# p768lwy3/torecsys

Measured on AMD Instinct MI355X. Metric: CTR samples/sec fwd+bwd (DeepFM, 39 fields x dim 64), higher is better.
Workload: dtype bf16; 1 GPU; BASELINE.json configs[1]: DeepFM 39 Criteo-shaped fields, MLP [400,400,400], 1000000 total rows, embed_dim 64, batch 65536, uniform indices, uniform field sizes; global_batch=65536, rows=1000000, parallelism=single, microbatches=1, optimizer=none, hipgraph=True, hipgraph_input_sets=1, hipgraph_steps_per_replay=4, fused_lookup_fm=True

## Files before the change

### include/trs_abi.h

```cpp
#ifndef TRS_ABI_H_
#define TRS_ABI_H_

#include <stddef.h>
#include <stdint.h>

#ifdef __cplusplus
extern "C" {
#endif

#define TRS_ABI_VERSION 3

enum { TRS_F32 = 0, TRS_BF16 = 1 };
enum { TRS_I64 = 0, TRS_I32 = 1 };
enum {
  TRS_OK = 0,
  TRS_EINVAL = -1,
  TRS_EDTYPE = -2,
  TRS_ESHAPE = -3,
  TRS_EALIGN = -4,
  TRS_ELAUNCH = -5,
  TRS_EWORKSPACE = -6
};

typedef void* trs_stream_t;
// ... 413 lines not shown
                      int64_t B, int32_t L, const void* w_qk, const void* b_qk, int32_t H, int32_t mode,
                      const void* gout, void* dx, float* dw_part, float* db_part, int32_t blocks, void* workspace,
                      size_t ws_bytes, int32_t* err_flag, trs_stream_t stream);

int trs_attn_pool_ragged_blocks(int64_t B, int32_t max_len, int32_t E, int32_t H, int32_t dtype, int32_t backward);
size_t trs_attn_pool_ragged_bwd_workspace_bytes(int32_t blocks, int32_t max_len, int32_t E, int32_t H);
int trs_attn_pool_ragged_fwd(const void* table, int64_t V, int32_t E, int32_t dtype, const void* ids, int32_t ids_dtype,
                             int64_t n, const void* offsets, int32_t off_dtype, int64_t n_off, int64_t B, int32_t max_len,
                             int64_t exclude_row, const void* w_qk, const void* b_qk, int32_t H, int32_t mode, void* out,
                             float* cnt, int32_t* err_flag, trs_stream_t stream);
int trs_attn_pool_ragged_bwd(const void* table, int64_t V, int32_t E, int32_t dtype, const void* ids, int32_t ids_dtype,
                             int64_t n, const void* offsets, int32_t off_dtype, int64_t n_off, int64_t B, int32_t max_len,
                             int64_t exclude_row, const void* w_qk, const void* b_qk, int32_t H, int32_t mode,
                             const void* gout, void* dx, float* dw_part, float* db_part, int32_t blocks, void* workspace,
                             size_t ws_bytes, int32_t* err_flag, trs_stream_t stream);

int trs_self_attn_path(int32_t L, int32_t E, int32_t H, int32_t dtype);
int trs_self_attn_blocks(int64_t B, int32_t L, int32_t E, int32_t H, int32_t dtype, int32_t backward);
size_t trs_self_attn_bwd_workspace_bytes(int32_t blocks, int32_t E);
int trs_self_attn_fwd(const void* x, int64_t B, int32_t L, int32_t E, int32_t H, int32_t dtype, const void* w_in,
                      const void* b_in, const void* w_out, const void* b_out, void* y, trs_stream_t stream);
int trs_self_attn_bwd(const void* x, int64_t B, int32_t L, int32_t E, int32_t H, int32_t dtype, const void* w_in,
                      const void* b_in, const void* w_out, const void* b_out, const void* gout, void* dx,
                      void* workspace, size_t ws_bytes, int32_t blocks, trs_stream_t stream);

int trs_dynamic_routing_path(int32_t N, int32_t R, int32_t K, int32_t dtype);
int trs_dynamic_routing_fwd(const float* priors, const void* noise, int64_t B, int32_t N, int32_t R, int32_t K,
                            int32_t num_iter, int32_t dtype, void* out, float* c_out, float* z_out, trs_stream_t stream);
int trs_dynamic_routing_bwd(const void* noise, const float* c, const float* z, const void* gout, int64_t B, int32_t N,
                            int32_t R, int32_t K, int32_t dtype, void* dpri, trs_stream_t stream);

int trs_seq_rnn_path(int32_t cell, int32_t L, int32_t E, int32_t dtype);
size_t trs_seq_rnn_workspace_bytes(int32_t cell, int32_t E);
int trs_seq_rnn_fwd(const void* table, int64_t V, int32_t E, int32_t dtype, const void* idx, int32_t idx_dtype,
                    const void* lengths, int32_t len_dtype, int64_t B, int32_t L, const void* w_ih, const void* w_hh,
                    const void* b_ih, const void* b_hh, int32_t cell, int32_t mode, int32_t average, float* scale,
                    void* out, void* h_save, float* c_save, void* workspace, size_t ws_bytes, int32_t* err_flag,
                    trs_stream_t stream);
int trs_seq_rnn_bwd(const void* table, int64_t V, int32_t E, int32_t dtype, const void* idx, int32_t idx_dtype,
                    const void* lengths, int32_t len_dtype, int64_t B, int32_t L, const void* w_ih, const void* w_hh,
                    const void* b_ih, const void* b_hh, int32_t cell, int32_t mode, const float* scale,
                    const void* h_save, const float* c_save, const void* gout, void* dgates, void* dgates_h,
                    void* workspace, size_t ws_bytes, trs_stream_t stream);

int trs_pack_columns(const void* const* srcs, const int32_t* widths, int32_t nsrc, int32_t src_dtype,
                     int64_t B, void* out, int32_t out_dtype, trs_stream_t stream);

int trs_ctr_logit_fwd(const void* fm, int32_t E, const void* feat, int32_t N, const void* const* extras,
                      const int64_t* extra_strides, int32_t n_extras, const void* bias, int64_t B, int32_t dtype,
                      void* out, trs_stream_t stream);
size_t trs_bce_logits_workspace_bytes(int64_t B);
int trs_bce_logits_fwd(const void* logits, int32_t dtype, const void* labels, int32_t label_dtype, int64_t B, float* loss,
                       void* workspace, size_t ws_bytes, trs_stream_t stream);
int trs_bce_logits_bwd(const void* logits, int32_t dtype, const void* labels, int32_t label_dtype, const float* gout,
                       int64_t B, void* glogits, trs_stream_t stream);

int trs_pair_score_path(int32_t E, int32_t dtype);
int trs_embed_pair_score_fwd(const void* a_table, int64_t Va, const void* a_idx, int64_t a_offset, const void* t_table,
                             int64_t Vt, const void* t_idx, int64_t t_offset, int32_t E, int32_t dtype, int32_t idx_dtype,
                             int64_t B, int32_t K, int32_t sim, void* scores, int32_t out_dtype, int32_t* err_flag,
                             trs_stream_t stream);
size_t trs_pair_score_bwd_workspace_bytes(int64_t B, int32_t K, int32_t E, int32_t dtype);
int trs_embed_pair_score_bwd(const void* a_table, int64_t Va, const void* a_idx, int64_t a_offset, const void* t_table,
                             int64_t Vt, const void* t_idx, int64_t t_offset, int32_t E, int32_t dtype, int32_t idx_dtype,
                             int64_t B, int32_t K, int32_t sim, const void* g_scores, int32_t g_dtype, void* g_block,
                             void* workspace, size_t ws_bytes, trs_stream_t stream);

size_t trs_rank_loss_workspace_bytes(int64_t B);
int trs_rank_loss_fwd(const void* pos, int64_t pos_stride, const void* neg, int64_t neg_stride, int32_t dtype,
                      const void* mask, int64_t B, int32_t K, int32_t kind, float margin, int32_t reduction, float* loss,
                      float* denom, void* workspace, size_t ws_bytes, trs_stream_t stream);
int trs_rank_loss_bwd(const void* pos, int64_t pos_stride, const void* neg, int64_t neg_stride, int32_t dtype,
                      const void* mask, int64_t B, int32_t K, int32_t kind, float margin, int32_t reduction,
                      const float* gout, const float* denom, void* g_pos, int64_t g_pos_stride, void* g_neg,
                      int64_t g_neg_stride, trs_stream_t stream);

#ifdef __cplusplus
}
#endif
#endif
```

### torecsys_amd/_abi.py

```python
from __future__ import annotations

import ctypes
import os
import threading
from ctypes import c_char_p, c_int32, c_int64, c_size_t, c_void_p

import torch

_HERE = os.path.dirname(os.path.abspath(__file__))
LIB_PATH = os.environ.get("TRS_LIB_PATH") or os.path.join(_HERE, "libtrs_hip.so")

TRS_F32, TRS_BF16 = 0, 1
TRS_I64, TRS_I32 = 0, 1

_P, _I32, _I64, _SZ, _F32 = c_void_p, c_int32, c_int64, c_size_t, ctypes.c_float

_OPTIMIZER_TAIL = [_I32, _F32, _P, _F32, _F32, _F32, _P, _P, _P, _SZ, _P]
_SR_TAIL = [ctypes.c_uint64, ctypes.c_uint64, _P]

SIGNATURES = {
    "trs_version": (c_int32, []),
    "trs_last_error_string": (c_char_p, []),
    "trs_rowdot_fwd": (c_int32, [_P, _P, _P, _I64, _I32, _I32, _P, _P]),
    "trs_rowdot_bwd_workspace_bytes": (_SZ, [_I64, _I32]),
# ... 123 lines not shown
    "trs_senet_scale_fwd": (c_int32, [_P, _P, _I64, _I32, _I32, _I32, _P, _P]),
    "trs_senet_scale_bwd": (c_int32, [_P, _P, _P, _P, _I64, _I32, _I32, _I32, _P, _P, _P]),
    "trs_moe_gate_vector_shape": (c_int32, [_I32, _I32]),
    "trs_moe_gate_last_path": (c_int32, []),
    "trs_moe_gate_fwd": (c_int32, [_P, _P, _P, _I64, _I32, _I32, _I32, _P, _P]),
    "trs_moe_gate_bwd": (c_int32, [_P, _P, _P, _P, _I64, _I32, _I32, _I32, _P, _P, _P]),
    "trs_dynamic_routing_path": (c_int32, [_I32, _I32, _I32, _I32]),
    "trs_dynamic_routing_fwd": (c_int32, [_P, _P, _I64, _I32, _I32, _I32, _I32, _I32, _P, _P, _P, _P]),
    "trs_dynamic_routing_bwd": (c_int32, [_P, _P, _P, _P, _I64, _I32, _I32, _I32, _I32, _P, _P]),
    "trs_seq_rnn_path": (c_int32, [_I32, _I32, _I32, _I32]),
    "trs_seq_rnn_workspace_bytes": (_SZ, [_I32, _I32]),
    "trs_seq_rnn_fwd": (c_int32, [_P, _I64, _I32, _I32, _P, _I32, _P, _I32, _I64, _I32, _P, _P, _P, _P, _I32, _I32, _I32, _P,
                                  _P, _P, _P, _P, _SZ, _P, _P]),
    "trs_seq_rnn_bwd": (c_int32, [_P, _I64, _I32, _I32, _P, _I32, _P, _I32, _I64, _I32, _P, _P, _P, _P, _I32, _I32, _P, _P,
                                  _P, _P, _P, _P, _P, _SZ, _P]),
    "trs_fm_fwd": (c_int32, [_P, _I64, _I32, _I32, _I32, _P, _P, _P]),
    "trs_fm_bwd": (c_int32, [_P, _P, _P, _I64, _I32, _I32, _I32, _P, _P]),
    "trs_pair_dot_fwd": (c_int32, [_P, _I64, _I32, _I32, _I32, _P, _P]),
    "trs_embed_pair_dot": (c_int32, [_P, _I64, _I32, _I32, _P, _I32, _P, _I64, _I32, _P, _P, _P, _P]),
    "trs_pair_dot_bwd": (c_int32, [_P, _P, _I64, _I32, _I32, _I32, _P, _P]),
    "trs_ffm_fwd": (c_int32, [_P, _I64, _I32, _I32, _I32, _P, _P]),
    "trs_ffm_bwd": (c_int32, [_P, _P, _I64, _I32, _I32, _I32, _P, _P]),
    "trs_ffm_fused_fwd": (c_int32, [_P, _I64, _I32, _I32, _P, _I32, _P, _I64, _I32, _P, _P, _P]),
    "trs_ffm_fused_bwd": (c_int32, [_P, _I64, _I32, _I32, _P, _I32, _P, _P, _P, _P, _I64, _I32, _P, _P, _P]),
    "trs_cross_workspace_bytes": (_SZ, [_I64, _I32, _I32, _I32]),
    "trs_cross_fwd": (c_int32, [_P, _P, _P, _I64, _I32, _I32, _I32, _P, _P, _SZ, _P]),
    "trs_cross_bwd": (c_int32, [_P, _P, _P, _P, _I64, _I32, _I32, _I32, _I32, _P, _P, _P, _P, _SZ, _P]),
    "trs_cin_fwd": (c_int32, [_P, _P, _P, _P, _I64, _I32, _I32, _I32, _I32, _I32, _P, _P, _P]),
    "trs_cin_bwd": (c_int32, [_P, _P, _P, _P, _I64, _I32, _I32, _I32, _I32, _I32, _P, _P, _P, _I32, _P]),
    "trs_cin_cl_workspace_bytes": (_SZ, [_I32, _I32, _I32]),
    "trs_cin_cl_fwd": (c_int32, [_P, _I32, _P, _I32, _P, _P, _I64, _I32, _I32, _I32, _I32, _I32, _I32, _P, _P, _SZ, _P]),
    "trs_cin_cl_bwd_data_workspace_bytes": (_SZ, [_I32, _I32, _I32]),
    "trs_cin_cl_bwd_data": (c_int32, [_P, _I32, _P, _I32, _P, _I32, _P, _I64, _I32, _I32, _I32, _I32, _I32, _I32, _P, _P,
                                      _I32, _P, _SZ, _P]),
    "trs_cin_dw_workspace_bytes": (_SZ, [_I64, _I32, _I32, _I32]),
    "trs_cin_dw": (c_int32, [_P, _I64, _P, _P, _I64, _I32, _I32, _I32, _I32, _I32, _I32, _P, _P, _SZ, _P]),
    "trs_relu_bwd_bias_workspace_bytes": (_SZ, [_I64, _I32]),
    "trs_relu_bwd_bias": (c_int32, [_P, _P, _I64, _I32, _I32, _P, _P, _P, _SZ, _P]),
    "trs_mlp_fused_supported": (c_int32, [_I32, _P]),
    "trs_mlp_fused_family": (c_int32, [_I32, _P, _I64, _I32]),
    "trs_mlp_fused_workspace_bytes": (_SZ, [_I32, _P]),
    "trs_mlp_fused_mask_bytes": (_SZ, [_I64]),
    "trs_mlp_fused_fwd": (c_int32, [_P, _I64, _I32, _P, _P, _P, _P, _P, _P, _P, _I32, _I32, _I32, _P, _SZ, _P]),
    "trs_mlp_fused_bwd_data": (c_int32, [_P, _I64, _I32, _P, _P, _P, _P, _P, _P, _P, _P, _I32, _I32, _P, _SZ, _P]),
    "trs_mlp_fused_bwd_wlast_part_bytes": (_SZ, [_I32, _P, _I64, _I32, _I32, _I32]),
    "trs_mlp_fused_bwd_data_wlast": (c_int32, [_P, _I32, _I64, _I32, _P, _P, _P, _P, _P, _P, _P, _P, _P, _I32, _I32, _P, _SZ, _P,
                                               _I32, _I32, _P, _SZ, _P]),
    "trs_mlp_fused_bwd_data_parts": (c_int32, [_P, _I32, _I64, _I32, _P, _P, _P, _P, _P, _P, _P, _I32, _I32, _P, _SZ, _P, _P,
                                               _P, _I32, _I32, _P, _SZ, _P]),
    "trs_colsum_parts_reduce": (c_int32, [_I32, _P, _P, _P, _I32, _P, _P]),
    "trs_ctr_logit_fwd": (c_int32, [_P, _I32, _P, _I32, _P, _P, _I32, _P, _I64, _I32, _P, _P]),
    "trs_bce_logits_workspace_bytes": (_SZ, [_I64]),
    "trs_bce_logits_fwd": (c_int32, [_P, _I32, _P, _I32, _I64, _P, _P, _SZ, _P]),
    "trs_bce_logits_bwd": (c_int32, [_P, _I32, _P, _I32, _P, _I64, _P, _P]),
    "trs_pair_score_path": (c_int32, [_I32, _I32]),
    "trs_embed_pair_score_fwd": (c_int32, [_P, _I64, _P, _I64, _P, _I64, _P, _I64, _I32, _I32, _I32, _I64, _I32, _I32, _P,
                                           _I32, _P, _P]),
    "trs_pair_score_bwd_workspace_bytes": (_SZ, [_I64, _I32, _I32, _I32]),
    "trs_embed_pair_score_bwd": (c_int32, [_P, _I64, _P, _I64, _P, _I64, _P, _I64, _I32, _I32, _I32, _I64, _I32, _I32, _P,
                                           _I32, _P, _P, _SZ, _P]),
    "trs_rank_loss_workspace_bytes": (_SZ, [_I64]),
    "trs_rank_loss_fwd": (c_int32, [_P, _I64, _P, _I64, _I32, _P, _I64, _I32, _I32, _F32, _I32, _P, _P, _P, _SZ, _P]),
    "trs_rank_loss_bwd": (c_int32, [_P, _I64, _P, _I64, _I32, _P, _I64, _I32, _I32, _F32, _I32, _P, _P, _P, _I64, _P, _I64,
                                    _P]),
    "trs_bucket_workspace_bytes": (_SZ, [_I64, _I32]),
    "trs_bucket_by_owner": (c_int32, [_P, _I32, _P, _I64, _I32, _I64, _I32, _P, _P, _P, _P, _P, _SZ, _P]),
    "trs_embed_fm_sharded": (c_int32, [_P, _I64, _P, _I64, _I64, _I32, _I32, _P, _P, _I32, _I32, _I64, _I32, _P, _P, _P, _P,
                                       _P]),
    "trs_permute_grad": (c_int32, [_P, _P, _P, _P, _P, _I64, _I32, _I32, _I32, _P, _P]),
    "trs_bag_route_count": (c_int32, [_P, _I32, _I64, _I32, _I64, _I64, _I32, _P, _P, _P]),
    "trs_bag_route_place": (c_int32, [_P, _I32, _I64, _I32, _I64, _I64, _I32, _P, _P, _I64, _P]),
    "trs_bag_pool_segments": (c_int32, [_P, _I64, _I32, _I32, _P, _I64, _P, _I64, _P, _P, _P]),
    "trs_bag_combine": (c_int32, [_P, _I32, _I64, _I32, _F32, _I32, _P, _P]),
    "trs_bag_expand_grad": (c_int32, [_P, _I32, _I32, _P, _I64, _P, _I64, _I64, _I64, _P, _P, _P]),
}

_lib = None
_lock = threading.Lock()


def load() -> ctypes.CDLL:
    global _lib
    if _lib is not None:
        return _lib
    with _lock:
        if _lib is not None:
            return _lib
        if not os.path.exists(LIB_PATH):
            raise RuntimeError(
                f"torecsys_amd: HIP library not built ({LIB_PATH} missing). Run "
                "`python -m torecsys_amd.build` (or __graft_entry__.build()). There is no CPU fallback.")
        lib = ctypes.CDLL(LIB_PATH)
        for name, (res, args) in SIGNATURES.items():
            try:
                fn = getattr(lib, name)
            except AttributeError as e:
                raise RuntimeError(f"torecsys_amd: {LIB_PATH} does not export {name}; rebuild it") from e
            fn.restype = res
            fn.argtypes = args
        _lib = lib
    return _lib


def last_error() -> str:
    s = load().trs_last_error_string()
    return s.decode("utf-8", "replace") if s else ""
# ... 180 lines not shown
```

### torecsys_amd/csrc/head.hip

```cpp
#include <algorithm>

#include "trs_common.hpp"

namespace trs {

constexpr int HEAD_MAX_EXTRAS = 4;
struct HeadExtras {
  const void* p[HEAD_MAX_EXTRAS];
  int64_t stride[HEAD_MAX_EXTRAS];
  int n;
};

template <typename T>
__global__ __launch_bounds__(256) void ctr_logit_kernel(const T* __restrict__ fm, int E, const T* __restrict__ feat, int N,
                                                        HeadExtras ex, const T* __restrict__ bias, int64_t B,
                                                        T* __restrict__ out) {
  const int lane = threadIdx.x & 15;
  const bool fm_vec = fm != nullptr && (E * (int)sizeof(T)) % 8 == 0 && (reinterpret_cast<uintptr_t>(fm) & 7u) == 0;
  const int64_t groups = (int64_t)gridDim.x * (blockDim.x >> 4);
  const float b0 = bias != nullptr ? to_f32(bias[0]) : 0.f;
  for (int64_t b = (int64_t)blockIdx.x * (blockDim.x >> 4) + (threadIdx.x >> 4); b < B; b += groups) {
    float acc = 0.f;
    if (fm != nullptr) {
      const T* r = fm + b * E;
      if (fm_vec) {
        constexpr int VE = 8 / (int)sizeof(T);
        for (int e = lane * VE; e < E; e += 16 * VE) {
          const uint2 u = *reinterpret_cast<const uint2*>(r + e);
          if constexpr (sizeof(T) == 2) {
            acc += __uint_as_float(u.x << 16) + __uint_as_float(u.x & 0xffff0000u) + __uint_as_float(u.y << 16) +
                   __uint_as_float(u.y & 0xffff0000u);
          } else {
            acc += __uint_as_float(u.x) + __uint_as_float(u.y);
          }
        }
      } else {
        for (int e = lane; e < E; e += 16) acc += to_f32(r[e]);
      }
    }
    if (feat != nullptr) {
      const T* r = feat + b * N;
      for (int n = lane; n < N; n += 16) acc += to_f32(r[n]);
    }
#pragma unroll
    for (int k = 0; k < HEAD_MAX_EXTRAS; ++k)
      if (k < ex.n && lane == k) acc += to_f32(static_cast<const T*>(ex.p[k])[b * ex.stride[k]]);
    acc += __shfl_xor(acc, 8, 16);
    acc += __shfl_xor(acc, 4, 16);
    acc += __shfl_xor(acc, 2, 16);
    acc += __shfl_xor(acc, 1, 16);
    if (lane == 0) out[b] = from_f32<T>(acc + b0);
  }
}

__device__ __forceinline__ float bce_term(float x, float y) {
  return fmaxf(x, 0.f) - x * y + log1pf(expf(-fabsf(x)));
}

constexpr int BCE_BLOCK = 256;
constexpr int BCE_MAX_BLOCKS = 256;

template <typename T, typename L>
__global__ __launch_bounds__(BCE_BLOCK) void bce_partial_kernel(const T* __restrict__ x, const L* __restrict__ y, int64_t B,
                                                                float* __restrict__ partial) {
  __shared__ float red[BCE_BLOCK / 64];
  float acc = 0.f;
  const int64_t stride = (int64_t)gridDim.x * BCE_BLOCK;
  for (int64_t i = (int64_t)blockIdx.x * BCE_BLOCK + threadIdx.x; i < B; i += stride)
    acc += bce_term(to_f32(x[i]), to_f32(y[i]));
  acc = group_sum_down<64>(acc);
  if ((threadIdx.x & 63) == 0) red[threadIdx.x >> 6] = acc;
  __syncthreads();
  if (threadIdx.x == 0) {
    float s = 0.f;
#pragma unroll
    for (int w = 0; w < BCE_BLOCK / 64; ++w) s += red[w];
    partial[blockIdx.x] = s;
  }
}

__global__ __launch_bounds__(64) void bce_finish_kernel(const float* __restrict__ partial, int n, float inv_B,
                                                        float* __restrict__ loss) {
  float acc = 0.f;
  for (int i = threadIdx.x; i < n; i += 64) acc += partial[i];
  acc = group_sum_down<64>(acc);
  if (threadIdx.x == 0) *loss = acc * inv_B;
}

constexpr int64_t BCE_ONE_MAX = 1 << 13;
template <typename T, typename L>
__global__ __launch_bounds__(1024) void bce_one_kernel(const T* __restrict__ x, const L* __restrict__ y, int64_t B,
                                                       float inv_B, float* __restrict__ loss) {
  __shared__ float red[16];
  float acc = 0.f;
  for (int64_t i = threadIdx.x; i < B; i += 1024) acc += bce_term(to_f32(x[i]), to_f32(y[i]));
  acc = group_sum_down<64>(acc);
  if ((threadIdx.x & 63) == 0) red[threadIdx.x >> 6] = acc;
  __syncthreads();
  if (threadIdx.x == 0) {
    float s = 0.f;
#pragma unroll
    for (int w = 0; w < 16; ++w) s += red[w];
    *loss = s * inv_B;
  }
}

template <typename T, typename L>
__global__ __launch_bounds__(256) void bce_bwd_kernel(const T* __restrict__ x, const L* __restrict__ y,
                                                      const float* __restrict__ gout, float inv_B, int64_t B,
                                                      T* __restrict__ gx) {
  const float g = (gout != nullptr ? *gout : 1.f) * inv_B;
  const int64_t stride = (int64_t)gridDim.x * blockDim.x;
  for (int64_t i = (int64_t)blockIdx.x * blockDim.x + threadIdx.x; i < B; i += stride) {
    const float xv = to_f32(x[i]);
    const float sg = 1.f / (1.f + expf(-xv));
    gx[i] = from_f32<T>((sg - to_f32(y[i])) * g);
  }
}

template <typename T>
static int bce_fwd_launch(const void* x, const void* y, int label_dtype, int64_t B, float* loss, float* ws, hipStream_t s) {
  if (B <= BCE_ONE_MAX) {
    if (label_dtype == TRS_F32)
      hipLaunchKernelGGL((bce_one_kernel<T, float>), dim3(1), dim3(1024), 0, s, (const T*)x, (const float*)y, B, 1.f / (float)B, loss);
    else
      hipLaunchKernelGGL((bce_one_kernel<T, bf16_t>), dim3(1), dim3(1024), 0, s, (const T*)x, (const bf16_t*)y, B, 1.f / (float)B, loss);
    return check_launch("bce_logits_fwd");
  }
  const int blocks = (int)std::min<int64_t>(BCE_MAX_BLOCKS, (B + BCE_BLOCK * 4 - 1) / (BCE_BLOCK * 4));
  if (label_dtype == TRS_F32)
    hipLaunchKernelGGL((bce_partial_kernel<T, float>), dim3(blocks), dim3(BCE_BLOCK), 0, s, (const T*)x, (const float*)y, B, ws);
  else
    hipLaunchKernelGGL((bce_partial_kernel<T, bf16_t>), dim3(blocks), dim3(BCE_BLOCK), 0, s, (const T*)x, (const bf16_t*)y, B, ws);
  hipLaunchKernelGGL(bce_finish_kernel, dim3(1), dim3(64), 0, s, ws, blocks, 1.f / (float)B, loss);
  return check_launch("bce_logits_fwd");
}

template <typename T>
static int bce_bwd_launch(const void* x, const void* y, int label_dtype, const float* gout, int64_t B, void* gx,
                          hipStream_t s) {
  const int blocks = stream_grid(B, 256, 1024);
  if (label_dtype == TRS_F32)
    hipLaunchKernelGGL((bce_bwd_kernel<T, float>), dim3(blocks), dim3(256), 0, s, (const T*)x, (const float*)y, gout,
                       1.f / (float)B, B, (T*)gx);
  else
    hipLaunchKernelGGL((bce_bwd_kernel<T, bf16_t>), dim3(blocks), dim3(256), 0, s, (const T*)x, (const bf16_t*)y, gout,
                       1.f / (float)B, B, (T*)gx);
  return check_launch("bce_logits_bwd");
}

}

using namespace trs;

extern "C" int trs_ctr_logit_fwd(const void* fm, int32_t E, const void* feat, int32_t N, const void* const* extras,
                                 const int64_t* extra_strides, int32_t n_extras, const void* bias, int64_t B,
                                 int32_t dtype, void* out, trs_stream_t stream) {
  TRS_REQUIRE(dtype == TRS_F32 || dtype == TRS_BF16, TRS_EDTYPE, "ctr_logit_fwd: dtype %d", dtype);
  TRS_REQUIRE(n_extras >= 0 && n_extras <= HEAD_MAX_EXTRAS, TRS_ESHAPE, "ctr_logit_fwd: at most %d extra columns", HEAD_MAX_EXTRAS);
  TRS_REQUIRE(B >= 0 && E >= 0 && N >= 0, TRS_ESHAPE, "ctr_logit_fwd: negative size");
  if (B == 0) return TRS_OK;
  TRS_REQUIRE(out != nullptr && (n_extras == 0 || (extras != nullptr && extra_strides != nullptr)), TRS_EINVAL,
              "ctr_logit_fwd: NULL pointer");
  HeadExtras ex;
  ex.n = n_extras;
  for (int k = 0; k < HEAD_MAX_EXTRAS; ++k) {
    ex.p[k] = k < n_extras ? extras[k] : nullptr;
    ex.stride[k] = k < n_extras ? extra_strides[k] : 0;
    TRS_REQUIRE(k >= n_extras || ex.p[k] != nullptr, TRS_EINVAL, "ctr_logit_fwd: NULL extra column %d", k);
  }
  hipStream_t s = (hipStream_t)stream;
  const int blocks = stream_grid(B, 16, 2048);
  if (dtype == TRS_F32)
    hipLaunchKernelGGL(ctr_logit_kernel<float>, dim3(blocks), dim3(256), 0, s, (const float*)(E > 0 ? fm : nullptr), E,
                       (const float*)(N > 0 ? feat : nullptr), N, ex, (const float*)bias, B, (float*)out);
  else
    hipLaunchKernelGGL(ctr_logit_kernel<bf16_t>, dim3(blocks), dim3(256), 0, s, (const bf16_t*)(E > 0 ? fm : nullptr), E,
                       (const bf16_t*)(N > 0 ? feat : nullptr), N, ex, (const bf16_t*)bias, B, (bf16_t*)out);
  return check_launch("ctr_logit_fwd");
}

extern "C" size_t trs_bce_logits_workspace_bytes(int64_t B) { return (size_t)BCE_MAX_BLOCKS * 4; }

extern "C" int trs_bce_logits_fwd(const void* logits, int32_t dtype, const void* labels, int32_t label_dtype, int64_t B,
                                  float* loss, void* workspace, size_t ws_bytes, trs_stream_t stream) {
  TRS_REQUIRE((dtype == TRS_F32 || dtype == TRS_BF16) && (label_dtype == TRS_F32 || label_dtype == TRS_BF16), TRS_EDTYPE,
              "bce_logits_fwd: dtype %d / %d", dtype, label_dtype);
  TRS_REQUIRE(B > 0, TRS_ESHAPE, "bce_logits_fwd: the mean over an empty batch is undefined");
  TRS_REQUIRE(logits && labels && loss && workspace, TRS_EINVAL, "bce_logits_fwd: NULL pointer");
  TRS_REQUIRE(ws_bytes >= trs_bce_logits_workspace_bytes(B), TRS_EWORKSPACE, "bce_logits_fwd: workspace too small");
  hipStream_t s = (hipStream_t)stream;
  return dtype == TRS_F32 ? bce_fwd_launch<float>(logits, labels, label_dtype, B, loss, (float*)workspace, s)
                          : bce_fwd_launch<bf16_t>(logits, labels, label_dtype, B, loss, (float*)workspace, s);
}

extern "C" int trs_bce_logits_bwd(const void* logits, int32_t dtype, const void* labels, int32_t label_dtype,
                                  const float* gout, int64_t B, void* glogits, trs_stream_t stream) {
  TRS_REQUIRE((dtype == TRS_F32 || dtype == TRS_BF16) && (label_dtype == TRS_F32 || label_dtype == TRS_BF16), TRS_EDTYPE,
              "bce_logits_bwd: dtype %d / %d", dtype, label_dtype);
  if (B == 0) return TRS_OK;
  TRS_REQUIRE(logits && labels && glogits, TRS_EINVAL, "bce_logits_bwd: NULL pointer");
  hipStream_t s = (hipStream_t)stream;
  return dtype == TRS_F32 ? bce_bwd_launch<float>(logits, labels, label_dtype, gout, B, glogits, s)
                          : bce_bwd_launch<bf16_t>(logits, labels, label_dtype, gout, B, glogits, s);
}
```

### torecsys_amd/csrc/mlp_fused.hip

```cpp
#include <algorithm>

#include "trs_common.hpp"

namespace trs {

typedef __attribute__((ext_vector_type(8))) __bf16 mf_bf16x8;
typedef __attribute__((ext_vector_type(4))) float mf_f32x4;
typedef __attribute__((ext_vector_type(4))) unsigned mf_u32x4;

constexpr int MF_ROWS = 128;
constexpr int MF_MT = MF_ROWS / 16;
constexpr int MF_WAVES = 8;
constexpr int MF_MINW = 2;
constexpr int MF_MAXP = 2;
constexpr int MF_MAXL = 8;
constexpr int MF_MAXLIVE = 3;
constexpr int MF_MASK_TILE = 64 * MF_WAVES * 16;

__host__ __device__ __forceinline__ int mf_col_of_slot(int mt, int m) {
  return 32 * (mt >> 1) + 8 * (m >> 2) + 4 * (mt & 1) + (m & 3);
}

__global__ __launch_bounds__(256) void mlp_prepack_kernel(const bf16_t* __restrict__ W, const bf16_t* __restrict__ b,
                                                          int out_f, int in_f, int transpose, int NTt ,
                                                          int KS, bf16_t* __restrict__ Wf, float* __restrict__ bf,
                                                          int bias_n) {
  const int total = NTt * KS * 64;
  for (int t = blockIdx.x * blockDim.x + threadIdx.x; t < total; t += gridDim.x * blockDim.x) {
    const int lane = t & 63;
    const int f = t >> 6;
    const int ks = f % KS, mt = f / KS;
    const int oc = mf_col_of_slot(mt, lane & 15);
    const int k0 = 32 * ks + 8 * (lane >> 4);
#pragma unroll
    for (int j = 0; j < 8; ++j) {
      const int k = k0 + j;
      bf16_t v{0};
      if (!transpose) {
        if (oc < out_f && k < in_f) v = W[(size_t)oc * in_f + k];
      } else {
        if (oc < in_f && k < out_f) v = W[(size_t)k * in_f + oc];
      }
      Wf[(size_t)t * 8 + j] = v;
    }
  }
  if (bf != nullptr)
    for (int t = blockIdx.x * blockDim.x + threadIdx.x; t < bias_n; t += gridDim.x * blockDim.x)
      bf[t] = (b != nullptr && t < out_f) ? to_f32(b[t]) : 0.f;
}

struct MlpPackJob {
  const bf16_t* W;
  const bf16_t* b;
  bf16_t* Wf;
  float* bf;
  int out_f, in_f, NTt, KS, bias_n;
  int transpose;
};
struct MlpPackArgs {
  MlpPackJob job[MF_MAXL];
};
__global__ __launch_bounds__(256) void mlp_prepack_many_kernel(MlpPackArgs a) {
  const MlpPackJob& j = a.job[blockIdx.y];
  const int total = j.NTt * j.KS * 64;
  const int transpose = j.transpose;
  const bool vec = !transpose && (j.in_f & 7) == 0 && (reinterpret_cast<uintptr_t>(j.W) & 15u) == 0;
  for (int t = blockIdx.x * blockDim.x + threadIdx.x; t < total; t += gridDim.x * blockDim.x) {
    const int lane = t & 63;
    const int f = t >> 6;
    const int ks = f % j.KS, mt = f / j.KS;
    const int oc = mf_col_of_slot(mt, lane & 15);
    const int k0 = 32 * ks + 8 * (lane >> 4);
    uint4* dst = reinterpret_cast<uint4*>(j.Wf + (size_t)t * 8);
    if (vec) {
      *dst = (oc < j.out_f && k0 + 8 <= j.in_f) ? *reinterpret_cast<const uint4*>(j.W + (size_t)oc * j.in_f + k0)
                                                 : make_uint4(0, 0, 0, 0);
      continue;
    }
    uint16_t v[8];
#pragma unroll
    for (int e = 0; e < 8; ++e) {
      const int k = k0 + e;
      v[e] = 0;
      if (!transpose) {
        if (oc < j.out_f && k < j.in_f) v[e] = j.W[(size_t)oc * j.in_f + k].v;
      } else {
        if (oc < j.in_f && k < j.out_f) v[e] = j.W[(size_t)k * j.in_f + oc].v;
      }
    }
    *dst = make_uint4(v[0] | ((uint32_t)v[1] << 16), v[2] | ((uint32_t)v[3] << 16), v[4] | ((uint32_t)v[5] << 16),
                      v[6] | ((uint32_t)v[7] << 16));
  }
  if (j.bf != nullptr)
    for (int t = blockIdx.x * blockDim.x + threadIdx.x; t < j.bias_n; t += gridDim.x * blockDim.x)
      j.bf[t] = (j.b != nullptr && t < j.out_f) ? to_f32(j.b[t]) : 0.f;
}

struct MlpStep {
  const uint4* wf;
  const float* bias;
  void* out;
  uint8_t* mask;
  float* colsum;
  int K, N;
  int out_stride;
  int relu;
};
struct MlpArgs {
  MlpStep step[MF_MAXL];
  int nsteps;
  const void* in;
  int in_stride;
  int nbias;
  int64_t rows;
  int act_str;
  uint8_t* mask_in;
  float* colsum_in;
  int ro_masks;
  const void* h_last;
// ... 650 lines not shown
  float s = 0.f;
  if (i < n)
    for (int p = ty; p < nparts; p += 4) s += part[(size_t)p * n + i];
  red[ty][tx] = s;
  __syncthreads();
  if (ty == 0 && i < n) out[i] = (red[0][tx] + red[1][tx]) + (red[2][tx] + red[3][tx]);
}

constexpr int MF_GRID = 256;

static bool mlp_fused_covers(int L, const int32_t* w) {
  if (L < 1 || L > MF_MAXL) return false;
  for (int i = 0; i <= L; ++i)
    if (w[i] < 8 || w[i] % 8 != 0 || pad32(w[i]) > 32 * MF_MAXP * MF_WAVES) return false;
  return true;
}

int mlp_resolve_family(int L, const int32_t* widths, int64_t rows, int request);
size_t mlp_ro_mask_bytes(int64_t rows);
int mlp_ro_fwd(const void* x, int64_t rows, int L, const int32_t* widths, const void* const* weights,
               const void* const* biases, void* const* hidden, void* const* masks, void* mask_in, void* y, void* workspace,
               hipStream_t s, int x_stride);
struct RoColsum {
  const float* part[9];
  float* out[9];
  int n[9];
  int count, nparts;
};
int mlp_ro_bwd(const void* gy, int64_t rows, int L, const int32_t* widths, const void* const* weights,
               const void* const* masks, void* const* gz, float* const* gbias, void* gx, const void* mask_in,
               float* gbias_in, void* workspace, hipStream_t s, RoColsum* cs);

static int mlp_act_str(int L, const int32_t* w) {
  int mx = 0;
  for (int i = 0; i <= L; ++i) mx = std::max(mx, pad32(w[i]));
  return mx * 2 + 16;
}

static size_t mlp_frag_bytes(int L, const int32_t* w) {
  size_t b = 0;
  for (int l = 0; l < L; ++l) b += (size_t)pad32(w[l]) * pad32(w[l + 1]) * 2;
  return (b + 255) / 256 * 256;
}

static int mlp_fwd_pack_jobs(int L, const int32_t* widths, const void* const* weights, const void* const* biases, char* wsp,
                             MlpPackJob* job) {
  float* bias_base = (float*)(wsp + mlp_frag_bytes(L, widths));
  size_t woff = 0, boff = 0;
  int blocks = 1;
  for (int l = 0; l < L; ++l) {
    const int K = pad32(widths[l]), N = pad32(widths[l + 1]);
    job[l] = MlpPackJob{(const bf16_t*)weights[l], (const bf16_t*)biases[l], (bf16_t*)(wsp + woff), bias_base + boff,
                        widths[l + 1], widths[l], N / 16, K / 32, N, 0};
    blocks = std::max(blocks, std::min(256, (N / 16 * (K / 32) * 64 + 255) / 256));
    woff += (size_t)K * N * 2;
    boff += N;
  }
  return blocks;
}
static int mlp_bwd_pack_jobs(int L, const int32_t* widths, const void* const* weights, char* wsp, MlpPackJob* job) {
  size_t woff = 0;
  int blocks = 1;
  for (int sidx = 0; sidx < L; ++sidx) {
    const int l = L - 1 - sidx;
    const int K = pad32(widths[l + 1]), N = pad32(widths[l]);
    job[sidx] = MlpPackJob{(const bf16_t*)weights[l], nullptr, (bf16_t*)(wsp + woff), nullptr, widths[l + 1], widths[l],
                           N / 16, K / 32, 0, 1};
    blocks = std::max(blocks, std::min(256, (N / 16 * (K / 32) * 64 + 255) / 256));
    woff += (size_t)K * N * 2;
  }
  return blocks;
}
static int mlp_gemm_pack_job(const void* W, int out_f, int in_f, void* workspace, MlpPackJob* job) {
  const int K = pad32(out_f), N = pad32(in_f);
  job[0] = MlpPackJob{(const bf16_t*)W, nullptr, (bf16_t*)workspace, nullptr, out_f, in_f, N / 16, K / 32, 0, 1};
  return std::min(256, (N / 16 * (K / 32) * 64 + 255) / 256);
}

}

using namespace trs;

extern "C" size_t trs_mlp_fused_workspace_bytes(int32_t num_layers, const int32_t* widths) {
  if (!mlp_fused_covers(num_layers, widths)) return 0;
  size_t sum = 0;
  for (int l = 0; l <= num_layers; ++l) sum += (size_t)pad32(widths[l]);
  return mlp_frag_bytes(num_layers, widths) + (size_t)MF_GRID * 8 * sum * 4 + 4096;
}

extern "C" int32_t trs_mlp_fused_family(int32_t num_layers, const int32_t* widths, int64_t rows, int32_t request) {
  if (!mlp_fused_covers(num_layers, widths)) return 0;
  return mlp_resolve_family(num_layers, widths, rows, request);
}

extern "C" size_t trs_mlp_fused_mask_bytes(int64_t rows) {
  return std::max((size_t)((rows + MF_ROWS - 1) / MF_ROWS) * MF_MASK_TILE, mlp_ro_mask_bytes(rows));
}

extern "C" int trs_mlp_fused_supported(int32_t num_layers, const int32_t* widths) {
  if (!mlp_fused_covers(num_layers, widths)) return 0;
  const size_t lds = (size_t)MF_ROWS * mlp_act_str(num_layers, widths) + 8 * 512 * 4 +
                     (size_t)(num_layers + 1) * 512 * 4;
  return lds <= 160 * 1024 ? 1 : 0;
}

extern "C" int trs_mlp_fused_fwd(const void* x, int64_t rows, int32_t num_layers, const int32_t* widths,
                                 const void* const* weights, const void* const* biases, void* const* hidden,
                                 void* const* masks, void* mask_in, void* y, int32_t dtype, int32_t family,
                                 int32_t x_stride, void* workspace, size_t ws_bytes, trs_stream_t stream) {
  hipStream_t s = (hipStream_t)stream;
  TRS_REQUIRE(dtype == TRS_BF16, TRS_EDTYPE, "mlp_fused_fwd: bf16 only");
  TRS_REQUIRE(trs_mlp_fused_supported(num_layers, widths), TRS_ESHAPE, "mlp_fused_fwd: unsupported layer widths");
  TRS_REQUIRE(weights && biases && workspace && x && y && hidden && masks, TRS_EINVAL, "mlp_fused_fwd: NULL pointer");
  TRS_REQUIRE(ws_bytes >= trs_mlp_fused_workspace_bytes(num_layers, widths), TRS_EWORKSPACE,
              "mlp_fused_fwd: workspace too small");
  const int L = num_layers;
  const int fam = mlp_resolve_family(L, widths, rows, family);
  TRS_REQUIRE(fam != 0, TRS_EINVAL, "mlp_fused_fwd: kernel family %d is not available for this stack (trs_mlp_fused_family)", family);
  if (rows == 0) return TRS_OK;
  TRS_REQUIRE(x_stride == 0 || (x_stride >= widths[0] && x_stride % 8 == 0), TRS_ESHAPE, "mlp_fused_fwd: x_stride %d", x_stride);
  TRS_REQUIRE(x_stride == 0 || x_stride == widths[0] || fam != TRS_MLP_FAMILY_TILE, TRS_ESHAPE,
              "mlp_fused_fwd: rows wider than the stack's input (x_stride %d > %d) are read by the row-owner kernels only", x_stride, widths[0]);
  if (fam == TRS_MLP_FAMILY_ROW_OWNER || fam == TRS_MLP_FAMILY_MIXED)
    return mlp_ro_fwd(x, rows, L, widths, weights, biases, hidden, masks, mask_in, y, workspace, s,
                      x_stride ? x_stride : widths[0]);
  MlpArgs a;
  a.nsteps = L;
  a.in = x;
  a.in_stride = widths[0];
// ... 358 lines not shown
```

### torecsys_amd/functional.py

```python
from __future__ import annotations

import ctypes
import os
from typing import List, Optional, Sequence, Tuple

import torch
from torch.autograd import Function
from torch.autograd.function import once_differentiable

from . import _abi
from ._abi import call, index_dtype_code, ptr, require_device, size_query, stream_ptr, value_dtype_code

CHECK_INDICES = os.environ.get("TRS_CHECK_INDICES", "0") not in ("", "0")


def _as_index(idx: torch.Tensor) -> torch.Tensor:
    idx = idx.rename(None) if idx.has_names() else idx
    if idx.dtype not in (torch.int64, torch.int32):
        if idx.dtype.is_floating_point or idx.dtype == torch.bool:
            raise TypeError(f"indices must be an integer tensor, got {idx.dtype}")
        idx = idx.long()
    return idx.contiguous()


_lazy_flags = {}


class _ErrFlag:

    def __init__(self, dev):
        if CHECK_INDICES:
            self.t, self.lazy = torch.zeros(1, dtype=torch.int32, device=dev), False
        else:
            t = _lazy_flags.get(dev)
            if t is None:
                t = _lazy_flags[dev] = torch.zeros(1, dtype=torch.int32, device=dev)
            self.t, self.lazy = t, True

    def check(self, what):
        if not self.lazy and int(self.t.item()) != 0:
            raise IndexError(f"{what}: index out of range in self")


def index_errors_seen(device=None, reset: bool = True) -> bool:
    seen = False
    for dev, t in list(_lazy_flags.items()):
        if device is not None and torch.device(device) != dev:
            continue
        if int(t.item()) != 0:
            seen = True
            if reset:
                t.zero_()
    return seen


class RowBuckets:
    __slots__ = ("row_start", "perm", "V", "BN", "N", "ready", "stream")
# ... 3288 lines not shown
    return _FusedMLP.apply(x, *params)


class _CTRLogit(Function):

    @staticmethod
    def forward(ctx, fm, feat, bias, *extras):
        ref = fm if fm is not None else (feat if feat is not None else extras[0])
        require_device(ref, *[t for t in (fm, feat, bias, *extras) if t is not None])
        B = ref.shape[0]
        dt = ref.dtype
        for t in (fm, feat, bias, *extras):
            if t is not None and t.dtype != dt:
                raise ValueError("ctr_logit: every operand must have the same dtype")
        fmc = None if fm is None else fm.contiguous()
        ftc = None if feat is None else feat.reshape(B, -1).contiguous()
        E = 0 if fmc is None else fmc.shape[1]
        N = 0 if ftc is None else ftc.shape[1]
        cols, strides = [], []
        for t in extras:
            if t.dim() != 2 or t.shape[0] != B or t.shape[1] != 1:
                raise ValueError(f"ctr_logit: extra terms must be (B,1), got {tuple(t.shape)}")
            cols.append(t)
            strides.append(t.stride(0))
        out = torch.empty(B, 1, dtype=dt, device=ref.device)
        call("trs_ctr_logit_fwd", ptr(fmc), E, ptr(ftc), N, _ptr_array(cols), (ctypes.c_int64 * max(1, len(cols)))(*strides),
             len(cols), ptr(bias), B, value_dtype_code(out), ptr(out), stream_ptr())
        ctx.shapes = (None if fm is None else tuple(fm.shape), None if feat is None else tuple(feat.shape),
                      None if bias is None else tuple(bias.shape), len(extras))
        return out

    @staticmethod
    @once_differentiable
    def backward(ctx, g):
        fm_shape, feat_shape, bias_shape, n_extras = ctx.shapes
        needs = ctx.needs_input_grad
        B = g.shape[0]
        g_fm = g.expand(fm_shape) if fm_shape is not None and needs[0] else None
        g_feat = None
        if feat_shape is not None and needs[1]:
            g_feat = g.reshape(B, *([1] * (len(feat_shape) - 1))).expand(feat_shape)
        g_bias = g.sum().reshape(bias_shape) if bias_shape is not None and needs[2] else None
        return (g_fm, g_feat, g_bias, *[g if needs[3 + k] else None for k in range(n_extras)])


def ctr_logit(fm: Optional[torch.Tensor] = None, feat: Optional[torch.Tensor] = None,
              extras: Sequence[torch.Tensor] = (), bias: Optional[torch.Tensor] = None) -> torch.Tensor:
    if fm is None and feat is None and not extras:
        raise ValueError("ctr_logit: nothing to sum")
    strip = lambda t: None if t is None else (t.rename(None) if t.has_names() else t)
    return _CTRLogit.apply(strip(fm), strip(feat), bias, *[strip(t) for t in extras])


class _BCEWithLogits(Function):
    @staticmethod
    def forward(ctx, logits, labels):
        require_device(logits, labels)
        x = logits.reshape(-1).contiguous()
        y = labels.reshape(-1).contiguous()
        if x.numel() != y.numel():
            raise ValueError(f"bce_with_logits: {tuple(logits.shape)} logits against {tuple(labels.shape)} labels")
        loss = torch.empty((), dtype=torch.float32, device=x.device)
        ws_bytes = size_query("trs_bce_logits_workspace_bytes", x.numel())
        ws = torch.empty(ws_bytes, dtype=torch.uint8, device=x.device)
        call("trs_bce_logits_fwd", ptr(x), value_dtype_code(x), ptr(y), value_dtype_code(y), x.numel(), ptr(loss), ptr(ws),
             ws_bytes, stream_ptr())
        ctx.save_for_backward(x, y)
        ctx.shape = tuple(logits.shape)
        return loss

    @staticmethod
    @once_differentiable
    def backward(ctx, g):
        x, y = ctx.saved_tensors
        gx = torch.empty_like(x)
        gf = g.float().contiguous()
        call("trs_bce_logits_bwd", ptr(x), value_dtype_code(x), ptr(y), value_dtype_code(y), ptr(gf), x.numel(), ptr(gx),
             stream_ptr())
        return gx.reshape(ctx.shape), None


def bce_with_logits(logits: torch.Tensor, labels: torch.Tensor) -> torch.Tensor:
    return _BCEWithLogits.apply(logits, labels)


PAIR_SIMS = {"dot": 0, "cosine": 1}
RANK_KINDS = {"pointwise": 0, "bpr": 1, "hinge": 2, "adaptive_hinge": 3}
RANK_REDUCTIONS = {"sum": 0, "mean": 1, "sample": 2}
PAIR_SCORE = os.environ.get("TRS_PAIR_SCORE", "1") not in ("", "0")


def pair_score_path(E: int, dtype: torch.dtype) -> int:
    if dtype not in (torch.float32, torch.bfloat16):
        return -1
    return size_query("trs_pair_score_path", int(E), _abi.TRS_F32 if dtype == torch.float32 else _abi.TRS_BF16)


def _sim_code(sim) -> int:
    if isinstance(sim, str):
        if sim not in PAIR_SIMS:
            raise ValueError(f"pair_scores: sim must be one of {sorted(PAIR_SIMS)}, got {sim!r}")
        return PAIR_SIMS[sim]
    if sim not in (0, 1):
        raise ValueError(f"pair_scores: bad sim code {sim!r}")
    return int(sim)


def _pair_operands(aw, a_idx, tw, t_idx, **more):
    named = dict(anchor_weight=aw, anchor_idx=a_idx, target_weight=tw, target_idx=t_idx, **more)
    for name, t in named.items():
        if t is not None and not t.is_contiguous():
            raise ValueError(f"pair_scores: {name} must be contiguous, got strides {tuple(t.stride())}")
    require_device(*named.values())
    if aw.dim() != 2 or tw.dim() != 2 or aw.shape[1] != tw.shape[1] or aw.dtype != tw.dtype:
        raise ValueError(f"pair_scores: two (V, E) tables of one dtype and width expected, got {tuple(aw.shape)} {aw.dtype} "
                         f"and {tuple(tw.shape)} {tw.dtype}")
    if a_idx.dim() != 1 or t_idx.dim() != 2 or t_idx.shape[0] != a_idx.shape[0] or t_idx.shape[1] < 1:
        raise ValueError(f"pair_scores: anchor ids (B,) and target ids (B, 1 + K) expected, got {tuple(a_idx.shape)} and "
                         f"{tuple(t_idx.shape)}")
# ... 277 lines not shown
```

Measured before the change: 63.10 million samples/s.

## Fuse BCE loss finish via last-block ticket; tile transposed MLP weight prepack

The BCE forward partial-sum kernel now uses an atomic ticket so the last block to finish reduces all partials and writes the mean loss, removing the separate single-block finish kernel launch. A per-device, per-stream ticket counter is allocated on the Python side and reset by the kernel itself. Separately, the transposed weight prepack for the fused MLP now stages 32x64 tiles through shared memory with coalesced 16-byte loads and a prefetch of the next tile, replacing scattered per-element reads. The ticket path adds threadfence and atomic overhead, and sharing one ticket between concurrent launches on the same stream relies on stream ordering.

```diff
diff --git a/include/trs_abi.h b/include/trs_abi.h
--- a/include/trs_abi.h
+++ b/include/trs_abi.h
@@ -489,6 +489,8 @@
 size_t trs_bce_logits_workspace_bytes(int64_t B);
 int trs_bce_logits_fwd(const void* logits, int32_t dtype, const void* labels, int32_t label_dtype, int64_t B, float* loss,
                        void* workspace, size_t ws_bytes, trs_stream_t stream);
+int trs_bce_logits_fwd_ticket(const void* logits, int32_t dtype, const void* labels, int32_t label_dtype, int64_t B,
+                              float* loss, void* workspace, size_t ws_bytes, int32_t* ticket, trs_stream_t stream);
 int trs_bce_logits_bwd(const void* logits, int32_t dtype, const void* labels, int32_t label_dtype, const float* gout,
                        int64_t B, void* glogits, trs_stream_t stream);
 
diff --git a/torecsys_amd/_abi.py b/torecsys_amd/_abi.py
--- a/torecsys_amd/_abi.py
+++ b/torecsys_amd/_abi.py
@@ -199,6 +199,7 @@
     "trs_ctr_logit_fwd": (c_int32, [_P, _I32, _P, _I32, _P, _P, _I32, _P, _I64, _I32, _P, _P]),
     "trs_bce_logits_workspace_bytes": (_SZ, [_I64]),
     "trs_bce_logits_fwd": (c_int32, [_P, _I32, _P, _I32, _I64, _P, _P, _SZ, _P]),
+    "trs_bce_logits_fwd_ticket": (c_int32, [_P, _I32, _P, _I32, _I64, _P, _P, _SZ, _P, _P]),
     "trs_bce_logits_bwd": (c_int32, [_P, _I32, _P, _I32, _P, _I64, _P, _P]),
     "trs_pair_score_path": (c_int32, [_I32, _I32]),
     "trs_embed_pair_score_fwd": (c_int32, [_P, _I64, _P, _I64, _P, _I64, _P, _I64, _I32, _I32, _I32, _I64, _I32, _I32, _P,
diff --git a/torecsys_amd/csrc/head.hip b/torecsys_amd/csrc/head.hip
--- a/torecsys_amd/csrc/head.hip
+++ b/torecsys_amd/csrc/head.hip
@@ -60,10 +60,12 @@
 constexpr int BCE_BLOCK = 256;
 constexpr int BCE_MAX_BLOCKS = 256;
 
-template <typename T, typename L>
+template <typename T, typename L, bool TICKET>
 __global__ __launch_bounds__(BCE_BLOCK) void bce_partial_kernel(const T* __restrict__ x, const L* __restrict__ y, int64_t B,
-                                                                float* __restrict__ partial) {
+                                                                float* partial, int32_t* ticket, float inv_B,
+                                                                float* __restrict__ loss) {
   __shared__ float red[BCE_BLOCK / 64];
+  __shared__ int last;
   float acc = 0.f;
   const int64_t stride = (int64_t)gridDim.x * BCE_BLOCK;
   for (int64_t i = (int64_t)blockIdx.x * BCE_BLOCK + threadIdx.x; i < B; i += stride)
@@ -76,6 +78,24 @@
 #pragma unroll
     for (int w = 0; w < BCE_BLOCK / 64; ++w) s += red[w];
     partial[blockIdx.x] = s;
+    if constexpr (TICKET) {
+      __threadfence();
+      last = __hip_atomic_fetch_add(ticket, 1, __ATOMIC_RELAXED, __HIP_MEMORY_SCOPE_AGENT) == (int)gridDim.x - 1;
+    }
+  }
+  if constexpr (TICKET) {
+    __syncthreads();
+    if (last && threadIdx.x < 64) {
+      __threadfence();
+      float acc = 0.f;
+      for (int i = threadIdx.x; i < (int)gridDim.x; i += 64)
+        acc += __hip_atomic_load(&partial[i], __ATOMIC_RELAXED, __HIP_MEMORY_SCOPE_AGENT);
+      acc = group_sum_down<64>(acc);
+      if (threadIdx.x == 0) {
+        *loss = acc * inv_B;
+        __hip_atomic_store(ticket, 0, __ATOMIC_RELAXED, __HIP_MEMORY_SCOPE_AGENT);
+      }
+    }
   }
 }
 
@@ -119,7 +139,8 @@
 }
 
 template <typename T>
-static int bce_fwd_launch(const void* x, const void* y, int label_dtype, int64_t B, float* loss, float* ws, hipStream_t s) {
+static int bce_fwd_launch(const void* x, const void* y, int label_dtype, int64_t B, float* loss, float* ws, int32_t* ticket,
+                          hipStream_t s) {
   if (B <= BCE_ONE_MAX) {
     if (label_dtype == TRS_F32)
       hipLaunchKernelGGL((bce_one_kernel<T, float>), dim3(1), dim3(1024), 0, s, (const T*)x, (const float*)y, B, 1.f / (float)B, loss);
@@ -128,11 +149,18 @@
     return check_launch("bce_logits_fwd");
   }
   const int blocks = (int)std::min<int64_t>(BCE_MAX_BLOCKS, (B + BCE_BLOCK * 4 - 1) / (BCE_BLOCK * 4));
-  if (label_dtype == TRS_F32)
-    hipLaunchKernelGGL((bce_partial_kernel<T, float>), dim3(blocks), dim3(BCE_BLOCK), 0, s, (const T*)x, (const float*)y, B, ws);
-  else
-    hipLaunchKernelGGL((bce_partial_kernel<T, bf16_t>), dim3(blocks), dim3(BCE_BLOCK), 0, s, (const T*)x, (const bf16_t*)y, B, ws);
-  hipLaunchKernelGGL(bce_finish_kernel, dim3(1), dim3(64), 0, s, ws, blocks, 1.f / (float)B, loss);
+  const float inv_B = 1.f / (float)B;
+  auto launch = [&](auto* kern, auto* labels) {
+    hipLaunchKernelGGL(kern, dim3(blocks), dim3(BCE_BLOCK), 0, s, (const T*)x, labels, B, ws, ticket, inv_B, loss);
+  };
+  if (ticket != nullptr) {
+    if (label_dtype == TRS_F32) launch(bce_partial_kernel<T, float, true>, (const float*)y);
+    else launch(bce_partial_kernel<T, bf16_t, true>, (const bf16_t*)y);
+    return check_launch("bce_logits_fwd_ticket");
+  }
+  if (label_dtype == TRS_F32) launch(bce_partial_kernel<T, float, false>, (const float*)y);
+  else launch(bce_partial_kernel<T, bf16_t, false>, (const bf16_t*)y);
+  hipLaunchKernelGGL(bce_finish_kernel, dim3(1), dim3(64), 0, s, ws, blocks, inv_B, loss);
   return check_launch("bce_logits_fwd");
 }
 
@@ -190,8 +218,22 @@
   TRS_REQUIRE(logits && labels && loss && workspace, TRS_EINVAL, "bce_logits_fwd: NULL pointer");
   TRS_REQUIRE(ws_bytes >= trs_bce_logits_workspace_bytes(B), TRS_EWORKSPACE, "bce_logits_fwd: workspace too small");
   hipStream_t s = (hipStream_t)stream;
-  return dtype == TRS_F32 ? bce_fwd_launch<float>(logits, labels, label_dtype, B, loss, (float*)workspace, s)
-                          : bce_fwd_launch<bf16_t>(logits, labels, label_dtype, B, loss, (float*)workspace, s);
+  return dtype == TRS_F32 ? bce_fwd_launch<float>(logits, labels, label_dtype, B, loss, (float*)workspace, nullptr, s)
+                          : bce_fwd_launch<bf16_t>(logits, labels, label_dtype, B, loss, (float*)workspace, nullptr, s);
+}
+
+extern "C" int trs_bce_logits_fwd_ticket(const void* logits, int32_t dtype, const void* labels, int32_t label_dtype,
+                                         int64_t B, float* loss, void* workspace, size_t ws_bytes, int32_t* ticket,
+                                         trs_stream_t stream) {
+  TRS_REQUIRE((dtype == TRS_F32 || dtype == TRS_BF16) && (label_dtype == TRS_F32 || label_dtype == TRS_BF16), TRS_EDTYPE,
+              "bce_logits_fwd_ticket: dtype %d / %d", dtype, label_dtype);
+  TRS_REQUIRE(B > 0, TRS_ESHAPE, "bce_logits_fwd_ticket: the mean over an empty batch is undefined");
+  TRS_REQUIRE(logits && labels && loss && workspace, TRS_EINVAL, "bce_logits_fwd_ticket: NULL pointer");
+  TRS_REQUIRE(ticket != nullptr, TRS_EINVAL, "bce_logits_fwd_ticket: NULL ticket");
+  TRS_REQUIRE(ws_bytes >= trs_bce_logits_workspace_bytes(B), TRS_EWORKSPACE, "bce_logits_fwd_ticket: workspace too small");
+  hipStream_t s = (hipStream_t)stream;
+  return dtype == TRS_F32 ? bce_fwd_launch<float>(logits, labels, label_dtype, B, loss, (float*)workspace, ticket, s)
+                          : bce_fwd_launch<bf16_t>(logits, labels, label_dtype, B, loss, (float*)workspace, ticket, s);
 }
 
 extern "C" int trs_bce_logits_bwd(const void* logits, int32_t dtype, const void* labels, int32_t label_dtype,
diff --git a/torecsys_amd/csrc/mlp_fused.hip b/torecsys_amd/csrc/mlp_fused.hip
--- a/torecsys_amd/csrc/mlp_fused.hip
+++ b/torecsys_amd/csrc/mlp_fused.hip
@@ -60,11 +60,46 @@
 struct MlpPackArgs {
   MlpPackJob job[MF_MAXL];
 };
+constexpr int MF_PK_PITCH = 68;
+inline int mlp_pack_blocks(int NTt, int KS, int transpose) {
+  return std::min(256, transpose ? (NTt + 3) / 4 * KS : (NTt * KS * 64 + 255) / 256);
+}
 __global__ __launch_bounds__(256) void mlp_prepack_many_kernel(MlpPackArgs a) {
   const MlpPackJob& j = a.job[blockIdx.y];
-  const int total = j.NTt * j.KS * 64;
   const int transpose = j.transpose;
-  const bool vec = !transpose && (j.in_f & 7) == 0 && (reinterpret_cast<uintptr_t>(j.W) & 15u) == 0;
+  const bool al = (j.in_f & 7) == 0 && (reinterpret_cast<uintptr_t>(j.W) & 15u) == 0;
+  const bool vec = !transpose && al, tiled = transpose && al;
+  const int total = tiled ? 0 : j.NTt * j.KS * 64;
+  __shared__ __attribute__((aligned(16))) uint16_t tile[32 * MF_PK_PITCH];
+  if (tiled) {
+    const int ntiles = (j.NTt + 3) / 4 * j.KS;
+    const int r = threadIdx.x >> 3, c8 = (threadIdx.x & 7) * 8;
+    const int mtl = threadIdx.x >> 6, lane = threadIdx.x & 63;
+    const uint16_t* col = tile + 8 * (lane >> 4) * MF_PK_PITCH + mf_col_of_slot(mtl, lane & 15);
+    auto load = [&](int tl) {
+      const int k = 32 * (tl % j.KS) + r, c = 64 * (tl / j.KS) + c8;
+      return (k < j.out_f && c + 8 <= j.in_f) ? *reinterpret_cast<const uint4*>(j.W + (size_t)k * j.in_f + c)
+                                               : make_uint4(0, 0, 0, 0);
+    };
+    int tl = blockIdx.x;
+    uint4 w = tl < ntiles ? load(tl) : make_uint4(0, 0, 0, 0);
+    for (; tl < ntiles; tl += gridDim.x) {
+      __syncthreads();
+      uint2* row = reinterpret_cast<uint2*>(tile + r * MF_PK_PITCH + c8);
+      row[0] = make_uint2(w.x, w.y);
+      row[1] = make_uint2(w.z, w.w);
+      __syncthreads();
+      const int ks = tl % j.KS, mt = 4 * (tl / j.KS) + mtl;
+      if (tl + (int)gridDim.x < ntiles) w = load(tl + gridDim.x);
+      if (mt < j.NTt) {
+        uint32_t v[8];
+#pragma unroll
+        for (int e = 0; e < 8; ++e) v[e] = col[e * MF_PK_PITCH];
+        reinterpret_cast<uint4*>(j.Wf)[(size_t)(mt * j.KS + ks) * 64 + lane] =
+            make_uint4(v[0] | (v[1] << 16), v[2] | (v[3] << 16), v[4] | (v[5] << 16), v[6] | (v[7] << 16));
+      }
+    }
+  }
   for (int t = blockIdx.x * blockDim.x + threadIdx.x; t < total; t += gridDim.x * blockDim.x) {
     const int lane = t & 63;
     const int f = t >> 6;
@@ -821,7 +856,7 @@
     const int K = pad32(widths[l]), N = pad32(widths[l + 1]);
     job[l] = MlpPackJob{(const bf16_t*)weights[l], (const bf16_t*)biases[l], (bf16_t*)(wsp + woff), bias_base + boff,
                         widths[l + 1], widths[l], N / 16, K / 32, N, 0};
-    blocks = std::max(blocks, std::min(256, (N / 16 * (K / 32) * 64 + 255) / 256));
+    blocks = std::max(blocks, mlp_pack_blocks(N / 16, K / 32, 0));
     woff += (size_t)K * N * 2;
     boff += N;
   }
@@ -835,7 +870,7 @@
     const int K = pad32(widths[l + 1]), N = pad32(widths[l]);
     job[sidx] = MlpPackJob{(const bf16_t*)weights[l], nullptr, (bf16_t*)(wsp + woff), nullptr, widths[l + 1], widths[l],
                            N / 16, K / 32, 0, 1};
-    blocks = std::max(blocks, std::min(256, (N / 16 * (K / 32) * 64 + 255) / 256));
+    blocks = std::max(blocks, mlp_pack_blocks(N / 16, K / 32, 1));
     woff += (size_t)K * N * 2;
   }
   return blocks;
@@ -843,7 +878,7 @@
 static int mlp_gemm_pack_job(const void* W, int out_f, int in_f, void* workspace, MlpPackJob* job) {
   const int K = pad32(out_f), N = pad32(in_f);
   job[0] = MlpPackJob{(const bf16_t*)W, nullptr, (bf16_t*)workspace, nullptr, out_f, in_f, N / 16, K / 32, 0, 1};
-  return std::min(256, (N / 16 * (K / 32) * 64 + 255) / 256);
+  return mlp_pack_blocks(N / 16, K / 32, 1);
 }
 
 }
diff --git a/torecsys_amd/functional.py b/torecsys_amd/functional.py
--- a/torecsys_amd/functional.py
+++ b/torecsys_amd/functional.py
@@ -2,7 +2,7 @@
 
 import ctypes
 import os
-from typing import List, Optional, Sequence, Tuple
+from typing import Dict, List, Optional, Sequence, Tuple
 
 import torch
 from torch.autograd import Function
@@ -3397,6 +3397,30 @@
     return _CTRLogit.apply(strip(fm), strip(feat), bias, *[strip(t) for t in extras])
 
 
+BCE_ONE_MAX = 1 << 13
+_BCE_TICKETS = 256
+_bce_ticket_block: Dict[int, torch.Tensor] = {}
+_bce_ticket_slot: Dict[Tuple[int, int], int] = {}
+
+
+def _bce_ticket(dev: torch.device) -> Optional[torch.Tensor]:
+    d = torch._C._cuda_getDevice()
+    block = _bce_ticket_block.get(d)
+    if block is None:
+        if torch.cuda.is_current_stream_capturing():
+            return None
+        block = _bce_ticket_block[d] = torch.zeros(_BCE_TICKETS, dtype=torch.int32, device=dev)
+        torch.cuda.current_stream(d).synchronize()
+    key = (d, int(torch._C._cuda_getCurrentRawStream(d)))
+    slot = _bce_ticket_slot.get(key)
+    if slot is None:
+        n = sum(1 for k in _bce_ticket_slot if k[0] == d)
+        if n >= _BCE_TICKETS:
+            return None
+        slot = _bce_ticket_slot[key] = n
+    return block[slot]
+
+
 class _BCEWithLogits(Function):
     @staticmethod
     def forward(ctx, logits, labels):
@@ -3408,8 +3432,13 @@
         loss = torch.empty((), dtype=torch.float32, device=x.device)
         ws_bytes = size_query("trs_bce_logits_workspace_bytes", x.numel())
         ws = torch.empty(ws_bytes, dtype=torch.uint8, device=x.device)
-        call("trs_bce_logits_fwd", ptr(x), value_dtype_code(x), ptr(y), value_dtype_code(y), x.numel(), ptr(loss), ptr(ws),
-             ws_bytes, stream_ptr())
+        ticket = _bce_ticket(x.device) if x.numel() > BCE_ONE_MAX else None
+        if ticket is not None:
+            call("trs_bce_logits_fwd_ticket", ptr(x), value_dtype_code(x), ptr(y), value_dtype_code(y), x.numel(), ptr(loss),
+                 ptr(ws), ws_bytes, ptr(ticket), stream_ptr())
+        else:
+            call("trs_bce_logits_fwd", ptr(x), value_dtype_code(x), ptr(y), value_dtype_code(y), x.numel(), ptr(loss), ptr(ws),
+                 ws_bytes, stream_ptr())
         ctx.save_for_backward(x, y)
         ctx.shape = tuple(logits.shape)
         return loss
```

New measurement: 63.62 million samples/s (median of 6 runs). About the same (+0.8%).
